# rcanut/nhwcodec

Hardware: AMD Instinct MI355X
Metric: encode Mpixels/s (512x512 RGB batch) (higher is better)
Workload: dtype int16

## Files before the change

nhwcodec_amd/csrc/nhw_enc.hip:

```cpp
#include "nhw_enc.h"

thread_local std::string nhw_enc_err;
extern "C" const char *nhw_last_error(void) { return nhw_enc_err.c_str(); }

static const size_t k_buf_bytes[B_COUNT] = {
	 8 * Q,  8 * Q,  Q,  Q,  2 * Q,  2 * Q,
	 2 * Q,  2 * Q,  Q / 2,  Q / 2,  4 * Q,  2 * Q,
	 2 * Q,  4 * Q + 256,  8 * Q,  16,  512,  6 * Q,
	 24832,  16384,  16384 + 256,  32768,  16384,  32768,
	 8192,  2 * Q + 1024,  2 * Q + 256,  2 * Q + 1024,  2 * Q + 1024,  Q / 2,
	 Q + 64, 8192 + 64, 16384 + 64,  Q + 64, 8192 + 64, 16384 + 64,  Q + 64, 8192 + 64, 16384 + 64,
	 2 * Q + 1024, 16384 + 64, 16384 + 64,  2048 + 64,  8 * Q + 64,
	 512,  512,  320000,  768,  768,  16384 + 64,  16384 + 64,
	 131072,  131072,  5632,  256,  512,  16,  16,  (8 + 9 * 512) * 2,
	 Q / 2 + 256,  Q / 2,  Q / 4,  4 * Q,
	 Q / 4 + 256,  2 * Q,
	 2 * Q,  2 * Q,  Q / 2,  Q / 2,  Q,
	 320 * 512
};

static size_t round_up(size_t v, size_t a) { return (v + a - 1) / a * a; }

extern "C" int nhw_quality_supported(int quality) { return quality >= 1 && quality <= 23; }

// ... 98 lines not shown
	const int rc = dev_alloc(host_set(e, (size_t)n), nullptr, n, nhw_enc_err);
	if (rc == NHW_OK) e->conv_cap = n;
	return rc;
}

#define STAGE_DONE() do { if (e->stop_after && ++stage == e->stop_after) { HIPCHK(hipGetLastError()); return NHW_OK; } } while (0)
static int chroma_head_launches(nhw_enc *e, const NhwWs &ws, int comp, int n, hipStream_t cs, int &stage)
{
	const int q = ws.q;
	const bool low = q <= 16;
	const bool vp = comp && ws.split_chroma;
	const Plane<int16_t> cjpeg = ws.plane<int16_t>(vp ? B_CJPEG_V : B_CJPEG), cproc = ws.plane<int16_t>(vp ? B_CPROC_V : B_CPROC);
	const Plane<int16_t> cll1 = ws.plane<int16_t>(vp ? B_CLL1_V : B_CLL1), cl2save = ws.plane<int16_t>(vp ? B_CL2SAVE_V : B_CL2SAVE);
	const Plane<const uint8_t> bytes = ws.plane<const uint8_t>(comp ? B_PV : B_PU);
	const bool widen_in_analysis = q > 14 && !ws.dbg;
	if (q <= 14) nhw_launch_low_prefilter_chroma(bytes, cjpeg, q, n, cs);
	else if (!widen_in_analysis) nhw_launch_phase(PH_C0, ws, comp, cs);
	STAGE_DONE();
	NhwAnalysis l1 = NhwAnalysis{ cjpeg, cproc, n, H, H, 0 }.saving(cll1, H / 2, ANA_SAVE_LL);
	l1.store = ws.dbg ? ANA_STORE_ALL : ANA_STORE_NO_T_LL_SAVED;
	if (widen_in_analysis) l1.src8 = bytes;
	nhw_launch_analysis(l1, cs);
	if (low) nhw_launch_low_chroma_thin(cproc, n, cs);
	STAGE_DONE();
	STAGE_DONE();
	if (!ws.dbg) {
		nhw_launch_chroma_loops(cproc, cll1, cl2save, ws.plane<const uint8_t>(B_PU), q, comp, ws.compat, n, cs);
		return 1;
	}
	const NhwAnalysis l2{ cjpeg, cproc, n, H, H / 2, 1 };
	nhw_launch_analysis(l2, cs);
	STAGE_DONE();
	nhw_launch_phase(PH_C2, ws, comp, cs);
	STAGE_DONE();
	nhw_launch_synthesis(cjpeg, cproc, n, H, H / 2, 0, cs);
	STAGE_DONE();
	nhw_launch_phase(PH_C3, ws, comp, cs);
	STAGE_DONE();
	nhw_launch_analysis(l2.saving(cl2save, H / 2, ANA_SAVE_BLOCK), cs);
	STAGE_DONE();
	STAGE_DONE();
	nhw_launch_phase(PH_C4, ws, comp, cs);
	STAGE_DONE();
	nhw_launch_synthesis(cjpeg, cproc, n, H, H / 2, 0, cs);
	STAGE_DONE();
	return 1;
}

static int luma_loop_launches(nhw_enc *e, const NhwWs &ws, int n, hipStream_t s, int &stage)
{
	const int q = ws.q;
	const Plane<int16_t> jpeg = ws.plane<int16_t>(B_JPEG), proc = ws.plane<int16_t>(B_PROC), ll1 = ws.plane<int16_t>(B_LL1), l2save = ws.plane<int16_t>(B_L2SAVE);
	const NhwAnalysis l2{ jpeg, proc, n, W, H, 1 };
	nhw_launch_analysis(l2.from(ll1, H), s);
	STAGE_DONE();
	if (q > 6) {
	nhw_launch_phase(PH_L1, ws, 0, s);
	nhw_launch_wave(WV_DQ1, ws, s);
	STAGE_DONE();
	if (ws.dbg) {
	nhw_launch_synthesis(jpeg, proc, n, W, H, 0, s);
	STAGE_DONE();
	nhw_launch_phase(PH_L2, ws, 0, s);
	STAGE_DONE();
	} else nhw_launch_l2_recon(jpeg, proc, ll1, q > 12 ? l2save : Plane<int16_t>{}, n, s);
	if (q <= 12) nhw_launch_analysis(l2, s);
	else if (ws.dbg) nhw_launch_analysis(l2.saving(l2save, H, ANA_SAVE_BLOCK), s);
	STAGE_DONE();
	}
	return 1;
}

static int run_batch(nhw_enc *e, const NhwWs &ws_in, const void *d_bgr, int n, int quality, void *d_out, uint32_t *d_sizes, int32_t *d_status, hipStream_t s,
                     int timed ,
                     int what = 3 )
{
	NhwWs ws = ws_in;
	const int q = quality;
	const bool low = q <= 16;
	const Plane<int16_t> jpeg = ws.plane<int16_t>(B_JPEG), proc = ws.plane<int16_t>(B_PROC);
	const Plane<uint8_t> pu = ws.plane<uint8_t>(B_PU), pv = ws.plane<uint8_t>(B_PV);

	e->low_parts_used = 1;
	int stage = 0;
	if (what & 1) {
	if (timed == 1) HIPCHK(hipEventRecord(e->ev[EV_START], s));
	const Plane<int16_t> yin = ws.plane<int16_t>(B_KMAP);
	NhwFront f;
	f.q = q; f.n = n; f.y = yin ; f.st = ws.plane<uint8_t>(B_ROWSTATE);
	f.proc = proc; f.jpeg = jpeg; f.ll1 = ws.plane<int16_t>(B_LL1); f.switches = ws.dbg ? 2 : 0;
	if (low) {
		nhw_launch_color((const uint8_t *)d_bgr, n, q, jpeg, pu, pv, s);
		HIPCHK(hipEventRecord(e->ev[EV_COLOR], s));
		STAGE_DONE();
		{ const int lparts = (timed == 1 && what == 3 && !e->stop_after && n >= 1024) ? e->low_parts : 1;
		  e->low_parts_used = lparts;
		  HIPCHK((hipError_t)nhw_launch_low_prefilter(jpeg, yin, proc, ws.plane<uint8_t>(B_SCAN), ws.plane<uint8_t>(B_KEEP), ws.plane<uint8_t>(B_LOWTAB), q, n, s, (e->front_fallback & 1) ? 32 : 0,
		                                              lparts, e->low_stream, e->low_ev)); }
		HIPCHK(hipEventRecord(e->ev[EV_PREFILTER], s));
		STAGE_DONE();
		if (ws.compat) nhw_launch_low_stale(proc, ws.plane<uint8_t>(B_STALE), n, s);
	} else {
		HIPCHK(hipEventRecord(e->ev[EV_COLOR], s)); HIPCHK(hipEventRecord(e->ev[EV_PREFILTER], s));
		STAGE_DONE();
		if (q < 22) STAGE_DONE();
		f.bgr = (const uint8_t *)d_bgr; f.pu = pu; f.pv = pv; f.with_prefilter = q < 22; f.switches |= e->front_fallback & 1;
		if (q > 21) f.keep = ws.plane<int16_t>(B_KEEP);
	}
	nhw_launch_front_fused(f, s);
	if (!low && ws.compat && q < 22) {
// ... 243 lines not shown
{
	if (!e || n < 1 || n > e->max_batch) { nhw_enc_err = "bad argument"; return NHW_E_ARG; }
	if (!e->timed || n > e->last_n || e->last_q < 15) {
		nhw_enc_err = "nhw_stage_chroma_l1: the handle's last batch does not cover the request (needs a completed batch of >= n images at quality >= 15)";
		return NHW_E_ARG;
	}
	HIPCHK(hipSetDevice(e->device));
	const NhwWs &ws = e->ws;
	hipStream_t s = stream ? (hipStream_t)stream : e->own_stream;
	HIPCHK(hipStreamWaitEvent(s, e->ev[EV_END], 0));
	NhwAnalysis l1 = NhwAnalysis{ ws.plane<int16_t>(B_CJPEG), ws.plane<int16_t>(B_CPROC), n, H, H, 0 }.saving(ws.plane<int16_t>(B_CLL1), H / 2, ANA_SAVE_LL);
	l1.store = ANA_STORE_NO_T_LL_SAVED;
	for (int comp = 0; comp < 2; comp++) { l1.src8 = ws.plane<const uint8_t>(comp ? B_PV : B_PU); nhw_launch_analysis(l1, s); }
	HIPCHK(hipGetLastError());
	return NHW_OK;
}

extern "C" int nhw_stage_chroma_loops(nhw_enc *e, int n, int comp, int form, void *stream)
{
	if (!e || n < 1 || n > e->max_batch || comp < 0 || comp > 1 || form < 0 || form > 8) { nhw_enc_err = "bad argument"; return NHW_E_ARG; }
	if (!e->timed || n > e->last_n || e->stop_after) {
		nhw_enc_err = "nhw_stage_chroma_loops: needs a completed whole batch of >= n images and no debug stop";
		return NHW_E_ARG;
	}
	HIPCHK(hipSetDevice(e->device));
	NhwWs ws = e->ws;
	ws.n = n; ws.q = e->last_q; ws.dbg = 0; ws.split_chroma = false;
	hipStream_t s = stream ? (hipStream_t)stream : e->own_stream;
	HIPCHK(hipStreamWaitEvent(s, e->ev[EV_END], 0));
	const Plane<int16_t> cjpeg = ws.plane<int16_t>(B_CJPEG), cproc = ws.plane<int16_t>(B_CPROC), cll1 = ws.plane<int16_t>(B_CLL1), cl2save = ws.plane<int16_t>(B_CL2SAVE);
	if (form == 0) {
		int stage = 0;
		const int rc = chroma_head_launches(e, ws, comp, n, s, stage);
		if (rc != 1) return rc;
	} else if (form == 1)
		nhw_launch_chroma_loops(cproc, cll1, cl2save, ws.plane<const uint8_t>(B_PU), ws.q, comp, ws.compat, n, s);
	else {
		const int k = form - 1;
		const NhwAnalysis l2{ cjpeg, cproc, n, H, H / 2, 1 };
		nhw_launch_analysis(l2.from(cll1, H / 2), s);
		if (k > 1) nhw_launch_phase(PH_C2, ws, comp, s);
		if (k > 2) nhw_launch_synthesis(cjpeg, cproc, n, H, H / 2, 0, s);
		if (k > 3) nhw_launch_phase(PH_C3, ws, comp, s);
		if (k > 4) nhw_launch_analysis(l2.saving(cl2save, H / 2, ANA_SAVE_BLOCK), s);
		if (k > 5) nhw_launch_phase(PH_C4, ws, comp, s);
		if (k > 6) nhw_launch_synthesis(cjpeg, cproc, n, H, H / 2, 0, s);
	}
	HIPCHK(hipGetLastError());
	return NHW_OK;
}

extern "C" int nhw_stage_luma_loop(nhw_enc *e, int n, int form, void *stream)
{
	if (!e || n < 1 || n > e->max_batch || form < 0 || form > 5) { nhw_enc_err = "bad argument"; return NHW_E_ARG; }
	if (!e->timed || n > e->last_n || e->stop_after || e->last_q < 7) {
		nhw_enc_err = "nhw_stage_luma_loop: needs a completed whole batch of >= n images at quality >= 7 and no debug stop";
		return NHW_E_ARG;
	}
	HIPCHK(hipSetDevice(e->device));
	NhwWs ws = e->ws;
	ws.n = n; ws.q = e->last_q; ws.dbg = 0;
	hipStream_t s = stream ? (hipStream_t)stream : e->own_stream;
	HIPCHK(hipStreamWaitEvent(s, e->ev[EV_END], 0));
	const Plane<int16_t> jpeg = ws.plane<int16_t>(B_JPEG), proc = ws.plane<int16_t>(B_PROC), ll1 = ws.plane<int16_t>(B_LL1), l2save = ws.plane<int16_t>(B_L2SAVE);
	const NhwAnalysis l2{ jpeg, proc, n, W, H, 1 };
	const bool save = ws.q > 12;
	if (form == 0) {
		int stage = 0;
		const int rc = luma_loop_launches(e, ws, n, s, stage);
		if (rc != 1) return rc;
	} else if (form == 1) {
		nhw_launch_l2_recon(jpeg, proc, ll1, save ? l2save : Plane<int16_t>{}, n, s);
		if (!save) nhw_launch_analysis(l2, s);
	} else {
		if (form == 3 || form == 4) {
			nhw_launch_analysis(l2.from(ll1, H), s);
			nhw_launch_phase(PH_L1, ws, 0, s);
			nhw_launch_wave(WV_DQ1, ws, s);
		}
		nhw_launch_synthesis(jpeg, proc, n, W, H, 0, s);
		if (form < 4) {
			nhw_launch_phase(PH_L2, ws, 0, s);
			nhw_launch_analysis(save ? l2.saving(l2save, H, ANA_SAVE_BLOCK) : l2, s);
		}
	}
	HIPCHK(hipGetLastError());
	return NHW_OK;
}

extern "C" int nhw_stage_synthesis(nhw_enc *e, void *d_jpeg, void *d_proc, int n_img, size_t plane_stride, int stride, int size, void *stream)
{
	if (!e || n_img < 1) return NHW_E_ARG;
	if (size != 256 && size != 128) { nhw_enc_err = "synthesis: transform size must be 256 or 128 (the encoder has no synthesis of size 512)"; return NHW_E_ARG; }
	HIPCHK(hipSetDevice(e->device));
	nhw_launch_synthesis({ (int16_t *)d_jpeg, plane_stride }, { (int16_t *)d_proc, plane_stride }, n_img, stride, size, 0, stream ? (hipStream_t)stream : e->own_stream);
	HIPCHK(hipGetLastError());
	return NHW_OK;
}

extern "C" int nhw_debug_front_fallback(nhw_enc *e, int on) { if (!e) return NHW_E_ARG; e->front_fallback = on; return NHW_OK; }
extern "C" int nhw_debug_stop_after(nhw_enc *e, int stage) { if (!e) return NHW_E_ARG; e->stop_after = stage; return NHW_OK; }
extern "C" int nhw_debug_slice_order(nhw_enc *e, int mode) { if (!e || mode < 0 || mode > 2) return NHW_E_ARG; e->slice_order = mode; return NHW_OK; }
__global__ __launch_bounds__(256) void k_debug_hash(const uint8_t *base, size_t stride, size_t words, unsigned long long *out)
{
	const uint32_t *p = reinterpret_cast<const uint32_t *>(base + (size_t)blockIdx.x * stride);
	unsigned long long h = 0;
	for (size_t i = threadIdx.x; i < words; i += 256) {
		unsigned long long x = ((unsigned long long)p[i] + 0x9E3779B97F4A7C15ull) * (2 * i + 1);
		x ^= x >> 29; x *= 0xBF58476D1CE4E5B9ull; x ^= x >> 32;
		h += x;
	}
	if (threadIdx.x == 0) out[blockIdx.x] = 0;
	__syncthreads();
	atomicAdd(&out[blockIdx.x], h);
}
extern "C" int nhw_debug_hash(nhw_enc *e, int buf, size_t bytes, int n, void *d_out, void *stream)
{
	if (!e || buf < 0 || buf >= B_COUNT || n < 1 || n > e->max_batch || bytes > e->ws.stride[buf]) return NHW_E_ARG;
	HIPCHK(hipSetDevice(e->device));
	k_debug_hash<<<n, 256, 0, stream ? (hipStream_t)stream : e->own_stream>>>(e->ws.base + e->ws.off[buf], e->ws.stride[buf], bytes / 4, (unsigned long long *)d_out);
	HIPCHK(hipGetLastError());
	return NHW_OK;
}
extern "C" int nhw_debug_fill(nhw_enc *e, int buf, int byte, size_t bytes, int n)
{
	if (!e || buf < 0 || buf >= B_COUNT || n < 1 || n > e->max_batch || bytes + GUARD > e->ws.stride[buf]) return NHW_E_ARG;
// ... 23 lines not shown
```

nhwcodec_amd/csrc/nhw_host.h:

```cpp
#ifndef NHW_HOST_H
#define NHW_HOST_H

#include <hip/hip_runtime.h>
#include <stdint.h>
#include <string>
#include <vector>

#include "../../include/nhw_hip.h"

struct NhwWs;

template <class T> struct Plane {
	T *p = nullptr; size_t pitch = 0;
	Plane at(size_t i) const { return { p + i * pitch, pitch }; }
	size_t bytes() const { return pitch * sizeof(T); }
	operator Plane<const T>() const { return { p, pitch }; }
};

extern thread_local int nhw_slice_mode;

struct NhwSliceScope {
	int saved;
	explicit NhwSliceScope(int mode) : saved(nhw_slice_mode) { nhw_slice_mode = mode; }
	~NhwSliceScope() { nhw_slice_mode = saved; }
};

template <typename F> inline void nhw_slices(int nslices, F &&launch)
{
	if (nhw_slice_mode == 1) for (int i = 0; i < nslices; i++) launch(i);
	else if (nhw_slice_mode == 2) for (int i = nslices - 1; i >= 0; i--) launch(i);
	else launch(-1);
}

void nhw_launch_color(const uint8_t *bgr, int n, int q, Plane<int16_t> y, Plane<uint8_t> u, Plane<uint8_t> v, hipStream_t s);
enum NhwAnaSave { ANA_SAVE_NONE, ANA_SAVE_BLOCK , ANA_SAVE_LL  };
enum NhwAnaStore { ANA_STORE_ALL, ANA_STORE_NO_T, ANA_STORE_NO_T_LL_SAVED };
struct NhwAnalysis {
	Plane<int16_t> jpeg, proc; int n, stride, size, final_level;
	Plane<int16_t> save = {}; int save_row = 0; NhwAnaSave save_kind = ANA_SAVE_NONE; NhwAnaStore store = ANA_STORE_ALL;
	Plane<const uint8_t> src8 = {}; Plane<const int16_t> alt = {}; int alt_stride = 0;
	NhwAnalysis from(Plane<const int16_t> p, int row) const { NhwAnalysis a = *this; a.alt = p; a.alt_stride = row; return a; }
	NhwAnalysis saving(Plane<int16_t> p, int row, NhwAnaSave kind) const { NhwAnalysis a = *this; a.save = p; a.save_row = row; a.save_kind = kind; return a; }
};
void nhw_launch_analysis(const NhwAnalysis &a, hipStream_t s);
void nhw_launch_synthesis(Plane<int16_t> jpeg, Plane<int16_t> proc, int n, int stride, int size, int drop_nat, Plane<const uint8_t> verb_list, Plane<const uint8_t> verb_len, hipStream_t s);
inline void nhw_launch_synthesis(Plane<int16_t> jpeg, Plane<int16_t> proc, int n, int stride, int size, int drop_nat, hipStream_t s) { nhw_launch_synthesis(jpeg, proc, n, stride, size, drop_nat, {}, {}, s); }
void nhw_launch_synth(uint8_t *bgr, int n, uint32_t seed_base, hipStream_t s);
struct NhwFront {
	const uint8_t *bgr = nullptr; Plane<uint8_t> pu = {}, pv = {}, st = {}; Plane<const int16_t> y = {};
	Plane<int16_t> proc = {}, jpeg = {}, ll1 = {}, keep = {}; int q = 0, with_prefilter = 0, n = 0, switches = 0;
};
void nhw_launch_front_fused(const NhwFront &f, hipStream_t s);
void nhw_launch_front_stale(Plane<const int16_t> y, Plane<const uint8_t> st, Plane<uint8_t> stale, int n, hipStream_t s);
int nhw_front_set_attrs(const char **where);
enum { PH_L1, PH_L2, PH_L3, PH_L4A, PH_C0, PH_C2, PH_C3, PH_C4, PH_C5, PH_L4B = 10, PH_L4C, PH_L4D, PH_LLC, PH_L4C2 };
enum { WV_DQ1, WV_DQ0, WV_EMIT, WV_QUANT };
void nhw_launch_phase(int ph, const NhwWs &ws, int comp, hipStream_t s);
void nhw_launch_final(const NhwWs &ws, uint8_t *out, uint32_t *sizes, int32_t *status, hipStream_t s);
void nhw_launch_wave(int ph, const NhwWs &ws, hipStream_t s);
void nhw_launch_l2_recon(Plane<int16_t> jpeg, Plane<int16_t> proc, Plane<int16_t> ll1, Plane<int16_t> l2save , int n, hipStream_t s);
void nhw_launch_chroma_loops(Plane<int16_t> cproc, Plane<int16_t> cll1, Plane<int16_t> cl2save, Plane<const uint8_t> pu, int q, int comp, int compat, int n, hipStream_t s);
void nhw_launch_copy_block(Plane<const int16_t> src, int src_row, Plane<int16_t> dst, int dst_row, int rows, int cols, int n, hipStream_t s);
int nhw_tail_set_attrs(const char **where);
enum { LOW_EV_START = 0, LOW_EV_COUNT = 13 };
inline int low_ev_pass_a(int p) { return 1 + p; }
inline int low_ev_done(int parts, int p) { return 1 + parts + p; }
int nhw_launch_low_prefilter(Plane<const int16_t> src, Plane<int16_t> y, Plane<int16_t> km, Plane<uint8_t> so, Plane<uint8_t> chain, Plane<uint8_t> tab,
                             int q, int n, hipStream_t s, int force, int parts, hipStream_t *aux, hipEvent_t *ev);
void nhw_launch_low_prefilter_chroma(Plane<const uint8_t> src, Plane<int16_t> dst, int q, int n, hipStream_t s);
void nhw_launch_low_chroma_thin(Plane<int16_t> plane, int n, hipStream_t s);
void nhw_launch_low_ll2(Plane<int16_t> proc, int q, int n, hipStream_t s);
void nhw_launch_low_stale(Plane<const int16_t> km, Plane<uint8_t> stale, int n, hipStream_t s);
void nhw_launch_fit_gather(const uint8_t *d_bgr, const int *idx, int m, uint8_t *staging, hipStream_t s);
void nhw_launch_fit_select(const int *idx, int m, const uint8_t *st_out, const uint32_t *st_sizes, const int32_t *st_status, const void *limit,
                           const int32_t *dec_status, const uint64_t *sse, int quality, int last, uint8_t *out, uint32_t *sizes, int32_t *status,
                           int32_t *qual, uint64_t *sse_out, uint8_t *open, hipStream_t s);
void nhw_launch_fit_compact(const uint8_t *open, const int *idx, int m, int *next, int *count, hipStream_t s);
hipError_t nhw_launch_sse(const uint8_t *a, const uint8_t *b, int n, uint64_t *sse, hipStream_t s);
hipError_t nhw_launch_tile_pad(const nhw_picture *d_pics, int n_pics, int tile0, int m, uint8_t *d_tiles, hipStream_t s);
hipError_t nhw_launch_untile_crop(const uint8_t *d_tiles, const nhw_picture *d_pics, int n_pics, int tile0, int m, int scale , hipStream_t s);
hipError_t nhw_launch_untile_region(const uint8_t *d_tiles, const nhw_region *d_regs, int n_regs, int tile0, int m, hipStream_t s);
hipError_t nhw_launch_sse_crop(const uint8_t *d_tiles, const nhw_picture *d_pics, int n_pics, int tile0, int m, uint64_t *d_sse, hipStream_t s);
size_t nhw_container_head(uint8_t *dst, uint32_t width, uint32_t height, const uint32_t *lens, int t);
int nhw_container_parse(const uint8_t *c, size_t len, uint32_t *width, uint32_t *height, int *tiles, const uint8_t **dir);
void nhw_dec_props(const nhw_dec *d, int *device, int *max_batch, int *stop_after);

int nhw_hip_error(std::string &err, hipError_t e, const char *file, int line, const char *call);
#define HIPCHK(x) do { hipError_t e_ = (x); if (e_ != hipSuccess) return nhw_hip_error(NHW_ERR, e_, __FILE__, __LINE__, #x); } while (0)

struct DevBuf { void **p; size_t bytes; };
using DevSet = std::vector<DevBuf>;
template <class T> inline DevBuf dev_buf(T *&p, size_t count) { return { (void **)&p, count * sizeof(T) }; }
void dev_free(const DevSet &set);
int dev_alloc(const DevSet &set, const char *what, int images, std::string &err);

struct GrowBuf {
	void *p; size_t cap;
	template <class T> T *as() const { return (T *)p; }
};
hipError_t nhw_grow(GrowBuf &b, size_t bytes);
void nhw_grow_free(GrowBuf &b);

#endif
```

nhwcodec_amd/csrc/nhw_tail.hip:

```cpp
#include "nhw_host.h"
#include "nhw_tail_par.h"
#include "nhw_dwt.h"

using namespace nhw;

#ifndef NHW_DENSE_STREAM
#define NHW_DENSE_STREAM 0
#endif

template <int PH>
__global__ __launch_bounds__(256) void k_phase(NhwWs ws, int comp)
{
	__shared__ int sh_counts[2];
	__shared__ int sh_pos[2 * NT + 2];
	__shared__ uint32_t sh_z[4 * Q / 16 / 32 + 4];
	extern __shared__ __attribute__((aligned(16))) int16_t dyn_lds[];
	const int img = blockIdx.x, tid = threadIdx.x;
	Ctx c;
	ctx_load(&c, ws, img, comp);
	if (PH == PH_L1) luma_p1_par(&c, tid, sh_pos);
	else if (PH == PH_L2) luma_p2_par(&c, tid, dyn_lds);
	else if (PH == PH_L3) luma_p3_par(&c, tid, sh_pos, sh_counts, dyn_lds, ws.q <= 12 || ws.dbg != 0);
	else if (PH == PH_L4A) luma_p4a_par(&c, tid, dyn_lds);
	else if (PH == PH_L4B) luma_p4b_par(&c, tid, sh_pos, dyn_lds);
// ... 176 lines not shown
				for (int k = 0; k < 4; k++) { st[k] = ytab[precomp_index(d[k], nb[k] + prev)]; prev = d[k] + st[k]; }
				int np = __shfl_up(prev, 1);
				if (!lane) np = first;
				if (!__any(np != prev_in)) break;
				prev_in = np;
			}
			uint2 w;
			w.x = (uint32_t)(uint16_t)(ov[0] + st[0]) | ((uint32_t)(uint16_t)(ov[1] + st[1]) << 16); w.y = (uint32_t)(uint16_t)(ov[2] + st[2]) | ((uint32_t)(uint16_t)(ov[3] + st[3]) << 16);
			if (!ANA) *reinterpret_cast<uint2 *>(jp + (size_t)r * W + c0) = w;
			else {
				int lo[2], hi[2];
				ana_row_quad(w.x, w.y, lane, lo, hi);
				int16_t *x = A + (2 * lane) * LS + r;
				x[0] = (int16_t)lo[0]; x[LS] = (int16_t)lo[1]; x[HLF * LS] = (int16_t)hi[0]; x[(HLF + 1) * LS] = (int16_t)hi[1];
			}
		}
		if (ANA) {
			lds_barrier();
			int16_t *save = saveb + (size_t)img * save_stride;
			const int rr = lane >> 5, c8 = lane & 31;
#pragma unroll 1
			for (int i = 0; i < 8; i++) {
				const int c = r0 + 2 * i;
				const uint32_t *g = reinterpret_cast<const uint32_t *>(A + (c + rr) * LS + 8 * c8);
				*reinterpret_cast<uint4 *>(jp + (size_t)(c + rr) * W + 8 * c8) = make_uint4(g[0], g[1], g[2], g[3]);
				uint32_t Ew[PPL], Ow[PPL];
				int lo[PPL][2], hi[PPL][2];
#pragma unroll
				for (int u = 0; u < PPL; u++) {
					const uint32_t a = reinterpret_cast<const uint32_t *>(A + c * LS)[lane + 64 * u], b = reinterpret_cast<const uint32_t *>(A + (c + 1) * LS)[lane + 64 * u];
					Ew[u] = (a & 0xFFFFu) | (b << 16); Ow[u] = (a >> 16) | (b & 0xFFFF0000u);
				}
				ana_col_pair<PPL, HLF>(Ew, Ow, c < HLF, lane, lo, hi);
				asm volatile("" ::: "memory");
#pragma unroll
				for (int h = 0; h < 2; h++) {
					int16_t *x = A + (c + h) * LS;
#pragma unroll
					for (int u = 0; u < PPL; u++) { x[lane + 64 * u] = (int16_t)lo[u][h]; x[HLF + lane + 64 * u] = (int16_t)hi[u][h]; }
				}
				asm volatile("" ::: "memory");
				const uint4 w = make_uint4(g[0], g[1], g[2], g[3]);
				*reinterpret_cast<uint4 *>(p + (size_t)(c + rr) * W + 8 * c8) = w;
				*reinterpret_cast<uint4 *>(save + (size_t)(c + rr) * H + 8 * c8) = w;
			}
		}
		lds_barrier();
	}
}
void nhw_launch_l2_recon(Plane<int16_t> jpeg, Plane<int16_t> proc, Plane<int16_t> ll1, Plane<int16_t> l2save , int n, hipStream_t s)
{
	assert(jpeg.pitch == proc.pitch);
	(l2save.p ? k_l2_recon<true> : k_l2_recon<false>)<<<n < 256 ? n : 256, 1024, H * (H + 2) * sizeof(int16_t) + 288, s>>>(jpeg.p, proc.p, jpeg.pitch, ll1.p, ll1.pitch, n, l2save.p, l2save.pitch);
}

__global__ __launch_bounds__(512) __attribute__((amdgpu_waves_per_eu(8, 8))) void k_chroma_loops(int16_t *__restrict__ cprocb, size_t plane_stride, int16_t *__restrict__ cll1b, size_t ll1_stride,
                                                      int16_t *__restrict__ saveb, size_t save_stride, const uint8_t *__restrict__ pub, size_t pu_stride,
                                                      int q, int comp, int compat)
{
	constexpr int S = H / 2, LS = S + 2, HLF = S / 2;
	__shared__ __attribute__((aligned(16))) int16_t A[S * LS];
	const int t = threadIdx.x, lane = t & 63, wv = t >> 6, img = blockIdx.x, r0 = wv * 16;
	int16_t *p = cprocb + (size_t)img * plane_stride, *o = cll1b + (size_t)img * ll1_stride, *save = saveb + (size_t)img * save_stride;
	const uint8_t *pu = pub + (size_t)img * pu_stride;
	const int behind = compat ? (int16_t)(pu[32768] | (pu[32769] << 8)) : 0;
	auto ll1_row = [&](int i) { return reinterpret_cast<const uint32_t *>(o + (size_t)(r0 + (i < 16 ? i : 15)) * S)[lane]; };
	uint32_t w0 = ll1_row(0), w1 = ll1_row(1), w2 = ll1_row(2), w3 = ll1_row(3);
	int side = 0;
	if (lane < 16) side = p[(size_t)(r0 + lane) * H + S];
	else if (lane == 16) side = wv < 7 ? o[(size_t)(r0 + 16) * S] : behind;
	if (t == 0) o[Q >> 2] = (int16_t)behind;
	auto ana_row = [&](int16_t *x, uint32_t w) {
		const uint32_t Dw[1] = { w };
		int lo[1], hi[1];
		ana_row_pair<1>(Dw, lane, lo, hi);
		x[lane] = (int16_t)lo[0]; x[HLF + lane] = (int16_t)hi[0];
	};
	auto columns = [&](const int loop , int16_t *out) {
		for (int i = 0; i < 8; i++) {
			const int c = r0 + 2 * i;
			uint32_t Ew[1], Ow[1];
			int lo[1][2], hi[1][2];
			Ew[0] = *reinterpret_cast<const uint32_t *>(A + (2 * lane) * LS + c); Ow[0] = *reinterpret_cast<const uint32_t *>(A + (2 * lane + 1) * LS + c);
			ana_col_pair<1, HLF>(Ew, Ow, c < HLF, lane, lo, hi);
			*reinterpret_cast<uint32_t *>(A + lane * LS + c) = (uint32_t)(uint16_t)lo[0][0] | ((uint32_t)(uint16_t)lo[0][1] << 16);
			*reinterpret_cast<uint32_t *>(A + (HLF + lane) * LS + c) = (uint32_t)(uint16_t)hi[0][0] | ((uint32_t)(uint16_t)hi[0][1] << 16);
			if (out)
#pragma unroll
				for (int h = 0; h < 2; h++) { int16_t *d = out + (size_t)(c + h) * S; d[lane] = (int16_t)lo[0][h]; d[HLF + lane] = (int16_t)hi[0][h]; }
		}
		for (int i = 0; i < 16; i++) {
			const int r = r0 + i, col0 = r < HLF ? HLF : 0;
			int16_t *x = A + r;
			int v[3] = { x[lane * LS], x[(HLF + lane) * LS], __builtin_amdgcn_readlane(side, i) };
			int ll = v[0];
			if (loop) {
				if (q <= 15) ll = (int16_t)((ll & 0xFFFC) + 1);
				else if ((r == 0) == (bool)(lane & 1)) ll = clear_bit0(ll);
			} else if (ll > 0 && ll < 256) ll = clear_bit0(ll);
			if (col0) v[0] = 0;
			uint64_t pair[2] = { 0, 0 };
			if (!loop) {
				const uint64_t m0 = __ballot(v[0] == -7 || v[0] == -8), m1 = __ballot(v[1] == -7 || v[1] == -8);
				const M4 m = M4{ { col0 ? 0 : m0, m1, 0, 0 } };
				const M4 fired = alt_runs(m & dn1(m) & col_range(col0, S - 2));
				const M4 both = fired | up1(fired);
// ... 53 lines not shown
	lds_barrier();
#pragma unroll 1
	for (int i = 0; i < 16; i++) {
		int e, od;
		syn_pair<S>(A + (r0 + i) * LS, 1, lane, true, &e, &od);
		reinterpret_cast<uint32_t *>(p + (size_t)(r0 + i) * H)[lane] = (uint32_t)(uint16_t)e | ((uint32_t)(uint16_t)od << 16);
	}
}
void nhw_launch_chroma_loops(Plane<int16_t> cproc, Plane<int16_t> cll1, Plane<int16_t> cl2save, Plane<const uint8_t> pu, int q, int comp, int compat, int n, hipStream_t s)
{
	k_chroma_loops<<<n, 512, 0, s>>>(cproc.p, cproc.pitch, cll1.p, cll1.pitch, cl2save.p, cl2save.pitch, pu.p, pu.pitch, q, comp, compat);
}

__global__ __launch_bounds__(256) void k_copy_block(const int16_t *__restrict__ src, size_t src_plane, int src_row,
                                                    int16_t *__restrict__ dst, size_t dst_plane, int dst_row, int rows, int cols)
{
	const int16_t *sp = src + (size_t)blockIdx.x * src_plane;
	int16_t *dp = dst + (size_t)blockIdx.x * dst_plane;
	const int per = cols >> 3, n = rows * per;
	for (int i0 = threadIdx.x; i0 < n; i0 += 4 * 256) {
		uint4 v[4];
#pragma unroll
		for (int u = 0; u < 4; u++) { const int i = i0 + u * 256; if (i < n) v[u] = reinterpret_cast<const uint4 *>(sp + (size_t)(i / per) * src_row)[i % per]; }
#pragma unroll
		for (int u = 0; u < 4; u++) { const int i = i0 + u * 256; if (i < n) reinterpret_cast<uint4 *>(dp + (size_t)(i / per) * dst_row)[i % per] = v[u]; }
	}
}

static size_t phase_lds(int ph)
{
	const size_t tile = (size_t)NT * TLS * sizeof(int16_t);
	switch (ph) {
	case PH_L2: return 3 * 32 * 33 + 32;
	case PH_L3: return LL_LDS_BYTES;
	case PH_LLC: return LLC_LDS_BYTES;
	case PH_L4A: return RF_LDS_BYTES > (NT + 2) * TLS * sizeof(int16_t) ? RF_LDS_BYTES : (size_t)(NT + 2) * TLS * sizeof(int16_t);
	case PH_L4B: return (size_t)(NT + 2) * TLS * sizeof(int16_t);
	case PH_L4C: return 0;
	case PH_L4D: return SL_LDS_BYTES;
	case PH_C5: return CQ_LDS_BYTES > 32 * 130 * 2 + (32 * 128 + 258) * 2 ? CQ_LDS_BYTES : 32 * 130 * 2 + (32 * 128 + 258) * 2;
	default: return 0;
	}
}

int nhw_tail_set_attrs(const char **where)
{
#define SETATTR(fn) do { const hipError_t e_ = hipFuncSetAttribute(reinterpret_cast<const void *>(&fn), hipFuncAttributeMaxDynamicSharedMemorySize, 100 << 10); \
                         if (e_ != hipSuccess) { *where = "hipFuncSetAttribute(" #fn ", MaxDynamicSharedMemorySize)"; return (int)e_; } } while (0)
	SETATTR(k_phase<PH_L1>); SETATTR(k_phase<PH_L2>); SETATTR(k_phase<PH_L3>); SETATTR(k_phase<PH_C5>);
	for (const void *fn : { reinterpret_cast<const void *>(&k_l2_recon<false>), reinterpret_cast<const void *>(&k_l2_recon<true>) }) {
		const hipError_t e_ = hipFuncSetAttribute(fn, hipFuncAttributeMaxDynamicSharedMemorySize, (int)(H * (H + 2) * sizeof(int16_t) + 288));
		if (e_ != hipSuccess) { *where = "hipFuncSetAttribute(k_l2_recon, MaxDynamicSharedMemorySize)"; return (int)e_; }
	}
#undef SETATTR
	return 0;
}

void nhw_launch_phase(int ph, const NhwWs &ws, int comp, hipStream_t s)
{
	const dim3 g(ws.n), b(256);
	const size_t lds = phase_lds(ph);
#define PHASE(P) case P: k_phase<P><<<g, b, lds, s>>>(ws, comp); break
	switch (ph) {
	PHASE(PH_L1); PHASE(PH_L2); PHASE(PH_L3);
	case PH_L4A: if (ws.q >= 17) k_l4a<<<g, b, lds, s>>>(ws); else k_phase<PH_L4A><<<g, b, lds, s>>>(ws, comp); break;
	PHASE(PH_L4B); PHASE(PH_L4C);
	case PH_L4D: if (NHW_DENSE_STREAM || ws.dbg) k_phase<PH_L4D><<<g, b, lds, s>>>(ws, comp); else k_y31<<<g, 512, lds, s>>>(ws); break;
	PHASE(PH_LLC); PHASE(PH_L4C2); PHASE(PH_C0); PHASE(PH_C2); PHASE(PH_C3); PHASE(PH_C4); PHASE(PH_C5);
	}
#undef PHASE
}
void nhw_launch_final(const NhwWs &ws, uint8_t *out, uint32_t *sizes, int32_t *status, hipStream_t s)
{
	k_final<<<ws.n, 256, PK_LDS_BYTES, s>>>(ws, out, sizes, status);
}

void nhw_launch_copy_block(Plane<const int16_t> src, int src_row, Plane<int16_t> dst, int dst_row, int rows, int cols, int n, hipStream_t s)
{
	if ((cols | src_row | dst_row) & 7 || (src.pitch | dst.pitch) & 7 || ((uintptr_t)src.p | (uintptr_t)dst.p) & 15) { fprintf(stderr, "nhw_launch_copy_block: block not 16-byte aligned\n"); abort(); }
	k_copy_block<<<n, 256, 0, s>>>(src.p, src.pitch, src_row, dst.p, dst.pitch, dst_row, rows, cols);
}
```

nhwcodec_amd/csrc/nhw_tail_par.h:

```cpp
#ifndef NHW_TAIL_PAR_H
#define NHW_TAIL_PAR_H

#include "nhw_tail_dev.h"
#include "nhw_tail_wave.h"

namespace nhw {

#define NT 256
#define BARRIER() __syncthreads()
#include "nhw_residual_rules.h"


DEV void tag_l2_details_par(Ctx *c, int tid)
{
	const int16_t *p = c->proc;
	for (int g = tid; g < Q / 8; g += NT) {
		const int r = g >> 5, j0 = (g & 31) * 8;
		if (r < H / 2 && j0 < H / 2) continue;
		const int at0 = r * W + j0;
		const uint4 pv = *reinterpret_cast<const uint4 *>(p + at0);
		uint4 cv = *reinterpret_cast<const uint4 *>(c->ll1 + r * H + j0);
		uint4 uv = make_uint4(0, 0, 0, 0), dv = uv;
		int u0 = 0, d7 = 0;
		if (r > 0) { uv = *reinterpret_cast<const uint4 *>(p + at0 - W); u0 = p[at0 - W - 1]; }
		dv = *reinterpret_cast<const uint4 *>(p + at0 + W); d7 = p[at0 + W + 8];
		const uint32_t uw[4] = { uv.x, uv.y, uv.z, uv.w }, dw[4] = { dv.x, dv.y, dv.z, dv.w };
		uint32_t pw[4] = { pv.x, pv.y, pv.z, pv.w }, cw[4] = { cv.x, cv.y, cv.z, cv.w }, aw[4] = { 0, 0, 0, 0 };
#pragma unroll
		for (int e = 0; e < 8; e++) {
			const int s = (int16_t)(pw[e >> 1] >> (16 * (e & 1))), at = at0 + e;
			const int up = e ? (int)(int16_t)(uw[(e - 1) >> 1] >> (16 * ((e - 1) & 1))) : u0;
			const int dn = e < 7 ? (int)(int16_t)(dw[(e + 1) >> 1] >> (16 * ((e + 1) & 1))) : d7;
			const bool neg_big = s < -7 && mult8_or_7(-s), neg_mid = s < -4 && s >= -7;
			const bool p24 = s >= 2 && s < 5, p24_hit = p24 && at >= W + 1 && at < 2 * Q - W - 1 && (up != 0 || dn != 0);
			const bool pos = s >= 0 && !p24, p01 = pos && (s & 7) < 2, p57 = pos && !p01 && s > 4 && s <= 7;
			const int add = (neg_big || p57) ? 16000 : (neg_mid || p24_hit || p01) ? 12000 : 0;
			aw[e >> 1] |= (uint32_t)add << (16 * (e & 1));
		}
		typedef unsigned short u16x2_ __attribute__((ext_vector_type(2)));
#pragma unroll
		for (int i = 0; i < 4; i++) cw[i] = __builtin_bit_cast(uint32_t, (u16x2_)(__builtin_bit_cast(u16x2_, cw[i]) + __builtin_bit_cast(u16x2_, aw[i])));
		*reinterpret_cast<uint4 *>(c->ll1 + r * H + j0) = make_uint4(cw[0], cw[1], cw[2], cw[3]);
	}
}

DEV void apply_tags_par(Ctx *c, int tid, int16_t *lds)
{
	int8_t *steps = reinterpret_cast<int8_t *>(lds);
	int16_t *p = c->proc, *o = c->ll1;
	auto tag_cell = [&](int tile, int k) {
		const int ty = tile >> 2, tx = tile & 3, type = k >> 10, rl = (k >> 5) & 31, jl = k & 31;
		const int r = 32 * tx + rl + (type >= 1 ? H / 2 : 0), j = 32 * ty + jl + (type != 1 ? H / 2 : 0);
		return o + r * H + j;
	};
	auto target = [&](int tile, int k) {
		const int ty = tile >> 2, tx = tile & 3, yl = k >> 5, xl = 2 * (k & 31);
		return reinterpret_cast<uint32_t *>(p + (64 * ty + yl) * W + 64 * tx + xl);
	};
	int16_t tg[12]; uint32_t tv[8];
#pragma unroll
	for (int u = 0; u < 12; u++) tg[u] = *tag_cell(0, tid + u * NT);
#pragma unroll
	for (int u = 0; u < 8; u++) tv[u] = *target(0, tid + u * NT);
	for (int tile = 0; tile < 16; tile++) {
#pragma unroll
		for (int u = 0; u < 12; u++) {
			const int k = tid + u * NT, type = k >> 10, rl = (k >> 5) & 31, jl = k & 31;
			int step = 0;
			if (tg[u] > 14000) { *tag_cell(tile, k) = (int16_t)(tg[u] - 16000); step = 1; }
			else if (tg[u] > 10000) { *tag_cell(tile, k) = (int16_t)(tg[u] - 12000); step = -1; }
			steps[(type * 32 + rl) * 33 + jl] = (int8_t)step;
		}
		uint32_t cur[8];
#pragma unroll
		for (int u = 0; u < 8; u++) cur[u] = tv[u];
		if (tile + 1 < 16) {
#pragma unroll
			for (int u = 0; u < 12; u++) tg[u] = *tag_cell(tile + 1, tid + u * NT);
#pragma unroll
			for (int u = 0; u < 8; u++) tv[u] = *target(tile + 1, tid + u * NT);
		}
		BARRIER();
		const int ty = tile >> 2;
#pragma unroll
		for (int u = 0; u < 8; u++) {
			const int k = tid + u * NT, yl = k >> 5, xl = 2 * (k & 31), yy = 64 * ty + yl;
			const int rl = xl >> 1, jl = yl >> 1;
			int s0 = 0, s1 = 0;
			if (yy & 1) { s0 = steps[(0 * 32 + rl) * 33 + jl]; s1 = steps[(2 * 32 + rl) * 33 + jl]; }
			else s1 = steps[(1 * 32 + rl) * 33 + jl];
			if (s0 | s1) {
				const uint32_t v = cur[u];
				*target(tile, k) = (uint32_t)(uint16_t)((int16_t)(v & 0xFFFF) + s0) | ((uint32_t)(uint16_t)((int16_t)(v >> 16) + s1) << 16);
			}
// ... 2688 lines not shown
```

profiles/make_design_table.py:

```python
import json, os, re, sys
ROOT = os.path.dirname(os.path.dirname(os.path.abspath(__file__)))
STATS = os.path.join(ROOT, "profiles", "round7_kernel_stats_1stream.txt")
PMC = os.path.join(ROOT, "profiles", "round7_pmc.json")
BATCHES = 7.0
PH = ["L1", "L2", "L3", "L4A", "C0", "C2", "C3", "C4", "C5", "FINAL", "L4B", "L4C", "L4D", "LLC", "L4C2"]
WV = ["DQ1", "DQ0", "EMIT", "QUANT"]
WHAT = {
    "k_front_image": "a1 + a2 + Y2 + Y3 fused: BGR24 -> Y, 4:2:0 chroma planes out, pre-filter (carry chained in the kernel), both directions of the level-1 analysis, LL copy; a workgroup walks an image (32 rows a band, 512 threads, 78 KB LDS)",
    "k_front_plain": "the same without the pre-filter (q >= 22; q <= 16 and the analysis stage from a luma plane): horizontal pass from registers, 64 rows a band",
    "k_dwt_ana<256>": "level-2 luma analysis of both closed loops (whole block in LDS, persistent workgroups); level-1 chroma analysis only for q <= 14 and the stage checks",
    "k_chroma_l1q": "level-1 chroma analysis from the 4:2:0 byte plane, a quarter of the 256 x 256 block to a workgroup (four a CU); its coefficients are part of SURVEY's 6 B/pixel",
    "k_dwt_ana<128>": "level-2 chroma analysis (only the tests' stage checks run it)",
    "k_chroma_loops": "both chroma closed loops of a component on one LDS residency of its level-2 block: analysis, simulation 1, synthesis, pre-compensation, analysis (+ cl2save), simulation 2, synthesis (four workgroups a CU)",
    "k_dwt_syn<256>": "level-2 luma synthesis of the second closed loop",
    "k_dwt_syn<128>": "level-2 chroma synthesis (only the tests' stage checks run it)",
    "k_l2_recon": "first closed loop: level-2 synthesis + Y8 (tags -> reconstruction) + Y9 (LL1 pre-compensation) on one LDS residency of the block",
    "L1": "Y5 tag level-2 details", "L2": "Y8, Y9 as a kernel of their own (only the tests' stage checks run it)", "L3": "Y16 LL2 coder (parse), on a stream of its own beside the second dequantiser simulation",
    "L4A": "Y19-Y23: small runs (wavefront per row), residual classification (one table-driven step for every kind) and coding (column walks on LDS tiles)",
    "L4B": "Y24, Y25 position lists + list packing", "L4C": "Y27 detail clean-up (a wavefront takes 64 consecutive rows, neighbours in registers; Y26 only for q >= 22)", "L4D": "Y31 rewrites, on the symbol LIST (non-zero map + values); leaves map and offsets in stream order",
    "L4C2": "Y29 (q >= 22): band reconstruction, half synthesis, res6 / char_res1 / qsetting3 lists",
    "C0": "chroma: copy", "C2": "chroma: dequantiser simulation 1", "C3": "chroma: tags", "C4": "chroma: dequantiser simulation 2",
    "C5": "chroma: marks (running-index fixed point), LL2 emission, quantiser (wavefront per row); V leaves the merged chroma stream as a list", "LLC": "Z1 chroma LL2 coder", "FINAL": "Z2 packetiser + container",
    "k_l4a": "Y19-Y23 of q >= 17: Y21 small runs (wavefront per row, rows in which nothing fires skipped), Y22 + Y23 as ONE column sweep on registers and class tables (eight workgroups a CU)",
    "k_y31": "Y31 rewrites on the symbol LIST (non-zero map + values), 512 threads an image; leaves map and offsets in stream order",
    "k_final": "Z2 packetiser (both parts from the symbol lists) + container; a kernel of its own at four wavefronts a SIMD",
    "DQ1": "a8 dequantiser simulation, first closed loop (wavefront per image)", "DQ0": "a8 dequantiser simulation, second closed loop",
    "EMIT": "Y14/Y15 LL2 emission", "QUANT": "Y28 luma quantiser + Y30: the symbols leave as a list in stream order (wavefront per image); reads the level-2 block from l2save (Y26)",
}


def label(name):
    m = re.match(r"void k_phase<(\d+)>", name)
    if m:
        return f"`k_phase<{PH[int(m.group(1))]}>`", WHAT.get(PH[int(m.group(1))], "")
    m = re.match(r"void k_wave<(\d+)>", name)
    if m:
        return f"`k_wave<{WV[int(m.group(1))]}>`", WHAT.get(WV[int(m.group(1))], "")
    short = name.replace("void ", "").replace("nhw::", "").split("(")[0]
    base = re.sub(r"<.*", "", short)
    return f"`{short}`", WHAT.get(short, WHAT.get(base, ""))


def table():
    pmc = json.load(open(PMC))
    rows, tot_ms, tot_gb = [], 0.0, 0.0
    for ln in open(STATS):
        m = re.match(r"(.{78})\s+(\d+)\s+([\d.]+)\s+([\d.]+)", ln)
        if not m or "at::" in ln or "rocclr" in ln or "k_synth" in ln:
            continue
        name = m.group(1).strip().split("(")[0]
        calls, total = int(m.group(2)), float(m.group(3))
        key = max((k for k in pmc if len(k.strip()) >= 5 and name.startswith(k.strip())), key=len, default=None)
        rd = wr = None
        if key and "FETCH_SIZE" in pmc[key] and "WRITE_SIZE" in pmc[key]:
            rd = 2 * pmc[key]["FETCH_SIZE"]["per_launch"] * 1024 / 1e9 * calls / BATCHES
            wr = pmc[key]["WRITE_SIZE"]["per_launch"] * 1024 / 1e9 * calls / BATCHES
        rows.append((total / BATCHES, name, calls / BATCHES, rd, wr))
        tot_ms += total / BATCHES; tot_gb += (rd or 0) + (wr or 0)
    out = ["| kernel | passes | launches | ms | HBM read + written, GB | TB/s |", "|---|---|---|---|---|---|"]
    for ms, name, calls, rd, wr in sorted(rows, reverse=True):
        lab, what = label(name)
        gb = f"{rd:.2f} + {wr:.2f}" if rd is not None else "n/a"
        tbs = f"{(rd + wr) / ms:.2f}" if rd is not None and ms else ""
        out.append(f"| {lab} | {what} | {calls:.0f} | {ms:.2f} | {gb} | {tbs} |")
    out.append(f"| **sum (one stream, nothing overlaps)** | | | **{tot_ms:.1f}** | **{tot_gb:.1f}** | |")
    return "\n".join(out)


# ... 13 lines not shown
```

Baseline: 62050.

## Fuse first level-2 luma analysis with Y5 detail tagging in one kernel

Adds k_l2_first, which runs the first level-2 luma analysis from ll1 and then the Y5 tagging of level-2 details on the block held in LDS, replacing a separate analysis launch plus the PH_L1 phase kernel. The goal is to avoid writing the transformed block to global memory and reading it back for tagging, and to drop one launch. It also prefetches the next image's ll1 rows into registers. The cost is a large 1024-thread kernel with heavy LDS use, and it is gated off in debug and compat modes.

```diff
diff --git a/nhwcodec_amd/csrc/nhw_enc.hip b/nhwcodec_amd/csrc/nhw_enc.hip
--- a/nhwcodec_amd/csrc/nhw_enc.hip
+++ b/nhwcodec_amd/csrc/nhw_enc.hip
@@ -174,10 +174,12 @@
 	const int q = ws.q;
 	const Plane<int16_t> jpeg = ws.plane<int16_t>(B_JPEG), proc = ws.plane<int16_t>(B_PROC), ll1 = ws.plane<int16_t>(B_LL1), l2save = ws.plane<int16_t>(B_L2SAVE);
 	const NhwAnalysis l2{ jpeg, proc, n, W, H, 1 };
-	nhw_launch_analysis(l2.from(ll1, H), s);
+	const bool first_fused = q > 6 && !ws.dbg && !ws.compat;
+	if (first_fused) nhw_launch_l2_first(jpeg, proc, ll1, n, s);
+	else nhw_launch_analysis(l2.from(ll1, H), s);
 	STAGE_DONE();
 	if (q > 6) {
-	nhw_launch_phase(PH_L1, ws, 0, s);
+	if (!first_fused) nhw_launch_phase(PH_L1, ws, 0, s);
 	nhw_launch_wave(WV_DQ1, ws, s);
 	STAGE_DONE();
 	if (ws.dbg) {
@@ -527,7 +529,7 @@
 
 extern "C" int nhw_stage_luma_loop(nhw_enc *e, int n, int form, void *stream)
 {
-	if (!e || n < 1 || n > e->max_batch || form < 0 || form > 5) { nhw_enc_err = "bad argument"; return NHW_E_ARG; }
+	if (!e || n < 1 || n > e->max_batch || form < 0 || form > 7) { nhw_enc_err = "bad argument"; return NHW_E_ARG; }
 	if (!e->timed || n > e->last_n || e->stop_after || e->last_q < 7) {
 		nhw_enc_err = "nhw_stage_luma_loop: needs a completed whole batch of >= n images at quality >= 7 and no debug stop";
 		return NHW_E_ARG;
@@ -547,6 +549,10 @@
 	} else if (form == 1) {
 		nhw_launch_l2_recon(jpeg, proc, ll1, save ? l2save : Plane<int16_t>{}, n, s);
 		if (!save) nhw_launch_analysis(l2, s);
+	} else if (form == 6) nhw_launch_l2_first(jpeg, proc, ll1, n, s);
+	else if (form == 7) {
+		nhw_launch_analysis(l2.from(ll1, H), s);
+		nhw_launch_phase(PH_L1, ws, 0, s);
 	} else {
 		if (form == 3 || form == 4) {
 			nhw_launch_analysis(l2.from(ll1, H), s);
diff --git a/nhwcodec_amd/csrc/nhw_host.h b/nhwcodec_amd/csrc/nhw_host.h
--- a/nhwcodec_amd/csrc/nhw_host.h
+++ b/nhwcodec_amd/csrc/nhw_host.h
@@ -58,6 +58,7 @@
 void nhw_launch_phase(int ph, const NhwWs &ws, int comp, hipStream_t s);
 void nhw_launch_final(const NhwWs &ws, uint8_t *out, uint32_t *sizes, int32_t *status, hipStream_t s);
 void nhw_launch_wave(int ph, const NhwWs &ws, hipStream_t s);
+void nhw_launch_l2_first(Plane<int16_t> jpeg, Plane<int16_t> proc, Plane<int16_t> ll1, int n, hipStream_t s);
 void nhw_launch_l2_recon(Plane<int16_t> jpeg, Plane<int16_t> proc, Plane<int16_t> ll1, Plane<int16_t> l2save , int n, hipStream_t s);
 void nhw_launch_chroma_loops(Plane<int16_t> cproc, Plane<int16_t> cll1, Plane<int16_t> cl2save, Plane<const uint8_t> pu, int q, int comp, int compat, int n, hipStream_t s);
 void nhw_launch_copy_block(Plane<const int16_t> src, int src_row, Plane<int16_t> dst, int dst_row, int rows, int cols, int n, hipStream_t s);
diff --git a/nhwcodec_amd/csrc/nhw_tail.hip b/nhwcodec_amd/csrc/nhw_tail.hip
--- a/nhwcodec_amd/csrc/nhw_tail.hip
+++ b/nhwcodec_amd/csrc/nhw_tail.hip
@@ -252,6 +252,99 @@
 {
 	assert(jpeg.pitch == proc.pitch);
 	(l2save.p ? k_l2_recon<true> : k_l2_recon<false>)<<<n < 256 ? n : 256, 1024, H * (H + 2) * sizeof(int16_t) + 288, s>>>(jpeg.p, proc.p, jpeg.pitch, ll1.p, ll1.pitch, n, l2save.p, l2save.pitch);
+}
+
+__global__ __launch_bounds__(1024) void k_l2_first(int16_t *__restrict__ jpegb, int16_t *__restrict__ procb, size_t plane_stride, int16_t *__restrict__ ll1b, size_t ll1_stride, int n)
+{
+	extern __shared__ __attribute__((aligned(16))) int16_t smem[];
+	constexpr int S = H, LS = S + 2, HLF = S / 2, PPL = HLF / 64;
+	const int t = threadIdx.x, lane = t & 63, wv = t >> 6, r0 = wv * 16, c0 = 4 * lane;
+	const int rr = lane >> 5, c8 = lane & 31;
+	const bool upper = wv < 8;
+	const bool tagging = !upper || c8 >= 16;
+	int16_t *A = smem;
+	uint2 pre[16];
+	if ((int)blockIdx.x < n) {
+		const int16_t *src = ll1b + (size_t)blockIdx.x * ll1_stride;
+#pragma unroll
+		for (int i = 0; i < 16; i++) pre[i] = *reinterpret_cast<const uint2 *>(src + (size_t)(r0 + i) * H + c0);
+	}
+	for (int img = blockIdx.x; img < n; img += gridDim.x) {
+		int16_t *jp = jpegb + (size_t)img * plane_stride, *p = procb + (size_t)img * plane_stride, *o = ll1b + (size_t)img * ll1_stride;
+#pragma unroll
+		for (int i = 0; i < 16; i++) {
+			int lo[2], hi[2];
+			ana_row_quad(pre[i].x, pre[i].y, lane, lo, hi);
+			int16_t *x = A + (2 * lane) * LS + r0 + i;
+			x[0] = (int16_t)lo[0]; x[LS] = (int16_t)lo[1]; x[HLF * LS] = (int16_t)hi[0]; x[(HLF + 1) * LS] = (int16_t)hi[1];
+		}
+		if (img + (int)gridDim.x < n) {
+			const int16_t *src = ll1b + (size_t)(img + gridDim.x) * ll1_stride;
+#pragma unroll
+			for (int i = 0; i < 16; i++) pre[i] = *reinterpret_cast<const uint2 *>(src + (size_t)(r0 + i) * H + c0);
+		}
+		int side = 0;
+		if (lane < 16) { if (!upper) side = p[(size_t)(r0 + lane - 1) * W - 1]; }
+		else if (lane < 32) side = p[(size_t)(r0 + lane - 16 + 1) * W + H];
+		lds_barrier();
+#pragma unroll 1
+		for (int i = 0; i < 8; i++) {
+			const int c = r0 + 2 * i;
+			const uint32_t *g = reinterpret_cast<const uint32_t *>(A + (c + rr) * LS + 8 * c8);
+			*reinterpret_cast<uint4 *>(jp + (size_t)(c + rr) * W + 8 * c8) = make_uint4(g[0], g[1], g[2], g[3]);
+			uint32_t Ew[PPL], Ow[PPL];
+			int lo[PPL][2], hi[PPL][2];
+#pragma unroll
+			for (int u = 0; u < PPL; u++) {
+				const uint32_t a = reinterpret_cast<const uint32_t *>(A + c * LS)[lane + 64 * u], b = reinterpret_cast<const uint32_t *>(A + (c + 1) * LS)[lane + 64 * u];
+				Ew[u] = (a & 0xFFFFu) | (b << 16); Ow[u] = (a >> 16) | (b & 0xFFFF0000u);
+			}
+			ana_col_pair<PPL, HLF>(Ew, Ow, c < HLF, lane, lo, hi);
+			asm volatile("" ::: "memory");
+#pragma unroll
+			for (int h = 0; h < 2; h++) {
+				int16_t *x = A + (c + h) * LS;
+#pragma unroll
+				for (int u = 0; u < PPL; u++) { x[lane + 64 * u] = (int16_t)lo[u][h]; x[HLF + lane + 64 * u] = (int16_t)hi[u][h]; }
+			}
+			asm volatile("" ::: "memory");
+			*reinterpret_cast<uint4 *>(p + (size_t)(c + rr) * W + 8 * c8) = make_uint4(g[0], g[1], g[2], g[3]);
+		}
+		auto ll1_cells = [&](int i) { return tagging ? *reinterpret_cast<const uint4 *>(o + (size_t)(r0 + 2 * i + rr) * H + 8 * c8) : make_uint4(0, 0, 0, 0); };
+		uint4 w0 = ll1_cells(0), w1 = ll1_cells(1), w2 = ll1_cells(2), w3 = ll1_cells(3);
+		lds_barrier();
+#pragma unroll 1
+		for (int i = 0; i < 8; i++) {
+			const int r = r0 + 2 * i + rr;
+			const uint4 cv = w0;
+			w0 = w1; w1 = w2; w2 = w3;
+			if (i + 4 < 8) w3 = ll1_cells(i + 4);
+			const int left = __shfl(side, 2 * i + rr), right = __shfl(side, 16 + 2 * i + rr);
+			if (!tagging) continue;
+			const uint32_t *g = reinterpret_cast<const uint32_t *>(A + r * LS + 8 * c8);
+			const uint32_t pw[4] = { g[0], g[1], g[2], g[3] };
+			uint32_t uw[4] = { 0, 0, 0, 0 }, dw[4] = { 0, 0, 0, 0 }, cw[4] = { cv.x, cv.y, cv.z, cv.w };
+			int u0 = 0, d7 = 0;
+			if (r > 0) {
+				const uint32_t *gu = g - LS / 2;
+				uw[0] = gu[0]; uw[1] = gu[1]; uw[2] = gu[2]; uw[3] = gu[3];
+				u0 = c8 ? (int)A[(r - 1) * LS + 8 * c8 - 1] : left;
+			}
+			if (r < S - 1) {
+				const uint32_t *gd = g + LS / 2;
+				dw[0] = gd[0]; dw[1] = gd[1]; dw[2] = gd[2]; dw[3] = gd[3];
+				d7 = c8 < 31 ? (int)A[(r + 1) * LS + 8 * c8 + 8] : right;
+			}
+			tag_l2_cells8(pw, uw, u0, dw, d7, r * W + 8 * c8, cw);
+			*reinterpret_cast<uint4 *>(o + (size_t)r * H + 8 * c8) = make_uint4(cw[0], cw[1], cw[2], cw[3]);
+		}
+		lds_barrier();
+	}
+}
+void nhw_launch_l2_first(Plane<int16_t> jpeg, Plane<int16_t> proc, Plane<int16_t> ll1, int n, hipStream_t s)
+{
+	assert(jpeg.pitch == proc.pitch);
+	k_l2_first<<<n < 256 ? n : 256, 1024, H * (H + 2) * sizeof(int16_t), s>>>(jpeg.p, proc.p, jpeg.pitch, ll1.p, ll1.pitch, n);
 }
 
 __global__ __launch_bounds__(512) __attribute__((amdgpu_waves_per_eu(8, 8))) void k_chroma_loops(int16_t *__restrict__ cprocb, size_t plane_stride, int16_t *__restrict__ cll1b, size_t ll1_stride,
@@ -411,6 +504,10 @@
 		const hipError_t e_ = hipFuncSetAttribute(fn, hipFuncAttributeMaxDynamicSharedMemorySize, (int)(H * (H + 2) * sizeof(int16_t) + 288));
 		if (e_ != hipSuccess) { *where = "hipFuncSetAttribute(k_l2_recon, MaxDynamicSharedMemorySize)"; return (int)e_; }
 	}
+	{
+		const hipError_t e_ = hipFuncSetAttribute(reinterpret_cast<const void *>(&k_l2_first), hipFuncAttributeMaxDynamicSharedMemorySize, (int)(H * (H + 2) * sizeof(int16_t)));
+		if (e_ != hipSuccess) { *where = "hipFuncSetAttribute(k_l2_first, MaxDynamicSharedMemorySize)"; return (int)e_; }
+	}
 #undef SETATTR
 	return 0;
 }
diff --git a/nhwcodec_amd/csrc/nhw_tail_par.h b/nhwcodec_amd/csrc/nhw_tail_par.h
--- a/nhwcodec_amd/csrc/nhw_tail_par.h
+++ b/nhwcodec_amd/csrc/nhw_tail_par.h
@@ -10,6 +10,25 @@
 #define BARRIER() __syncthreads()
 #include "nhw_residual_rules.h"
 
+
+DEV void tag_l2_cells8(const uint32_t (&pw)[4], const uint32_t (&uw)[4], int u0, const uint32_t (&dw)[4], int d7, int at0, uint32_t (&cw)[4])
+{
+	uint32_t aw[4] = { 0, 0, 0, 0 };
+#pragma unroll
+	for (int e = 0; e < 8; e++) {
+		const int s = (int16_t)(pw[e >> 1] >> (16 * (e & 1))), at = at0 + e;
+		const int up = e ? (int)(int16_t)(uw[(e - 1) >> 1] >> (16 * ((e - 1) & 1))) : u0;
+		const int dn = e < 7 ? (int)(int16_t)(dw[(e + 1) >> 1] >> (16 * ((e + 1) & 1))) : d7;
+		const bool neg_big = s < -7 && mult8_or_7(-s), neg_mid = s < -4 && s >= -7;
+		const bool p24 = s >= 2 && s < 5, p24_hit = p24 && at >= W + 1 && at < 2 * Q - W - 1 && (up != 0 || dn != 0);
+		const bool pos = s >= 0 && !p24, p01 = pos && (s & 7) < 2, p57 = pos && !p01 && s > 4 && s <= 7;
+		const int add = (neg_big || p57) ? 16000 : (neg_mid || p24_hit || p01) ? 12000 : 0;
+		aw[e >> 1] |= (uint32_t)add << (16 * (e & 1));
+	}
+	typedef unsigned short u16x2_ __attribute__((ext_vector_type(2)));
+#pragma unroll
+	for (int i = 0; i < 4; i++) cw[i] = __builtin_bit_cast(uint32_t, (u16x2_)(__builtin_bit_cast(u16x2_, cw[i]) + __builtin_bit_cast(u16x2_, aw[i])));
+}
 
 DEV void tag_l2_details_par(Ctx *c, int tid)
 {
@@ -19,27 +38,14 @@
 		if (r < H / 2 && j0 < H / 2) continue;
 		const int at0 = r * W + j0;
 		const uint4 pv = *reinterpret_cast<const uint4 *>(p + at0);
-		uint4 cv = *reinterpret_cast<const uint4 *>(c->ll1 + r * H + j0);
+		const uint4 cv = *reinterpret_cast<const uint4 *>(c->ll1 + r * H + j0);
 		uint4 uv = make_uint4(0, 0, 0, 0), dv = uv;
 		int u0 = 0, d7 = 0;
 		if (r > 0) { uv = *reinterpret_cast<const uint4 *>(p + at0 - W); u0 = p[at0 - W - 1]; }
 		dv = *reinterpret_cast<const uint4 *>(p + at0 + W); d7 = p[at0 + W + 8];
-		const uint32_t uw[4] = { uv.x, uv.y, uv.z, uv.w }, dw[4] = { dv.x, dv.y, dv.z, dv.w };
-		uint32_t pw[4] = { pv.x, pv.y, pv.z, pv.w }, cw[4] = { cv.x, cv.y, cv.z, cv.w }, aw[4] = { 0, 0, 0, 0 };
-#pragma unroll
-		for (int e = 0; e < 8; e++) {
-			const int s = (int16_t)(pw[e >> 1] >> (16 * (e & 1))), at = at0 + e;
-			const int up = e ? (int)(int16_t)(uw[(e - 1) >> 1] >> (16 * ((e - 1) & 1))) : u0;
-			const int dn = e < 7 ? (int)(int16_t)(dw[(e + 1) >> 1] >> (16 * ((e + 1) & 1))) : d7;
-			const bool neg_big = s < -7 && mult8_or_7(-s), neg_mid = s < -4 && s >= -7;
-			const bool p24 = s >= 2 && s < 5, p24_hit = p24 && at >= W + 1 && at < 2 * Q - W - 1 && (up != 0 || dn != 0);
-			const bool pos = s >= 0 && !p24, p01 = pos && (s & 7) < 2, p57 = pos && !p01 && s > 4 && s <= 7;
-			const int add = (neg_big || p57) ? 16000 : (neg_mid || p24_hit || p01) ? 12000 : 0;
-			aw[e >> 1] |= (uint32_t)add << (16 * (e & 1));
-		}
-		typedef unsigned short u16x2_ __attribute__((ext_vector_type(2)));
-#pragma unroll
-		for (int i = 0; i < 4; i++) cw[i] = __builtin_bit_cast(uint32_t, (u16x2_)(__builtin_bit_cast(u16x2_, cw[i]) + __builtin_bit_cast(u16x2_, aw[i])));
+		const uint32_t uw[4] = { uv.x, uv.y, uv.z, uv.w }, dw[4] = { dv.x, dv.y, dv.z, dv.w }, pw[4] = { pv.x, pv.y, pv.z, pv.w };
+		uint32_t cw[4] = { cv.x, cv.y, cv.z, cv.w };
+		tag_l2_cells8(pw, uw, u0, dw, d7, at0, cw);
 		*reinterpret_cast<uint4 *>(c->ll1 + r * H + j0) = make_uint4(cw[0], cw[1], cw[2], cw[3]);
 	}
 }
diff --git a/profiles/make_design_table.py b/profiles/make_design_table.py
--- a/profiles/make_design_table.py
+++ b/profiles/make_design_table.py
@@ -14,6 +14,7 @@
     "k_chroma_loops": "both chroma closed loops of a component on one LDS residency of its level-2 block: analysis, simulation 1, synthesis, pre-compensation, analysis (+ cl2save), simulation 2, synthesis (four workgroups a CU)",
     "k_dwt_syn<256>": "level-2 luma synthesis of the second closed loop",
     "k_dwt_syn<128>": "level-2 chroma synthesis (only the tests' stage checks run it)",
+    "k_l2_first": "first level-2 luma analysis (from ll1) + Y5 (tags of the level-2 details) on one LDS residency of the block",
     "k_l2_recon": "first closed loop: level-2 synthesis + Y8 (tags -> reconstruction) + Y9 (LL1 pre-compensation) on one LDS residency of the block",
     "L1": "Y5 tag level-2 details", "L2": "Y8, Y9 as a kernel of their own (only the tests' stage checks run it)", "L3": "Y16 LL2 coder (parse), on a stream of its own beside the second dequantiser simulation",
     "L4A": "Y19-Y23: small runs (wavefront per row), residual classification (one table-driven step for every kind) and coding (column walks on LDS tiles)",
```

New measurement: 62590, median of 6. No clear change (+0.9%).
